# aosprey/mckpp-f90

Measured on AMD Instinct MI355X. Metric: column-steps/s at 1e5 cols x 60 levels, 1/2/4/8 GPU; % HBM roofline, higher is better.
Workload: dtype f64

## Files before the change

### mckpp_f90_amd/api.py

```python
import ctypes as C

import numpy as np

NI, NJ = 890, 48

F_PROFILES, F_SAVED, F_SCALARS, F_DIAG = 1, 2, 4, 8
F_RESTART = F_PROFILES | F_SAVED | F_SCALARS
F_ALL = 0xF

ST_ZERO_PIVOT, ST_LONG_ITER, ST_RETRIED, ST_FAILED, ST_DODGY = 1, 2, 4, 8, 16

_dp = C.POINTER(C.c_double)
_ip = C.POINTER(C.c_int32)

_SWITCHES = [
    "LKPP", "LRI", "LDD", "L_SSref", "L_RELAX_SST", "L_RELAX_CALCONLY", "L_FCORR", "L_FCORR_WITHZ",
    "L_SFCORR", "L_SFCORR_WITHZ", "L_RELAX_SAL", "L_RELAX_OCNT", "L_NO_FREEZE", "L_NO_ISOTHERM",
    "L_DAMP_CURR", "clim_present",
]


class _ConstC(C.Structure):
    _fields_ = (
        [(n, C.c_int32) for n in ("nz", "nztmax", "nsflxs", "njdt", "itermax")]
# ... 212 lines not shown
    "mckpp_hip_status": _sig(_H, _ip, _i64p, _ip, twin=True),
    "mckpp_hip_ncolumns": _sig(_H, res=_i64, twin=True),
    "mckpp_hip_last_kernel_ms": _sig(_H, _dp, _ip),
    "mckpp_hip_last_launch_count": _sig(_H, res=_i32),
    "mckpp_hip_kernel_name": _sig(_H, res=C.c_char_p),
    "mckpp_hip_kernel_residency": _sig(_H, _ip, _ip, _ip, _i64p),
    "mckpp_hip_eos_batch": _sig(_H, _i64, *[_dp] * 7),
    "mckpp_hip_exp_batch": _sig(_H, _i64, _dp, _dp),
    "mckpp_hip_div_batch": _sig(_H, _i64, _dp, _dp, _dp),
    "mckpp_hip_multi_ndev": _sig(_H, res=_i32),
    "mckpp_hip_multi_ctx": _sig(_H, _i32, res=_H),
    "mckpp_hip_multi_gather": _sig(_H, _i32, _i32, _dp),
}


def _signatures():
    out = {}
    for name, (res, argtypes, twin) in _SIGNATURES.items():
        out[name] = (res, argtypes)
        if twin:
            out["mckpp_hip_multi_" + name[len("mckpp_hip_"):]] = (res, argtypes)
    return out


def _bind(lib):
    if getattr(lib, "_mckpp_bound", False):
        return lib
    for name, (res, argtypes) in _signatures().items():
        fn = getattr(lib, name, None)
        if fn is not None:
            fn.restype, fn.argtypes = res, argtypes
    lib._mckpp_bound = True
    return lib


def _lib():
    from . import load_library

    return _bind(load_library())


def build_compiler():
    return _lib().mckpp_hip_build_compiler().decode()
# ... 406 lines not shown
        f = np.ascontiguousarray(fields, dtype=np.int32)
        self._call("window_select", f.ctypes.data_as(_ip), len(f))

    def window_fetch(self, field, op, out):
        assert out.flags["F_CONTIGUOUS"] and out.dtype == np.float64
        self._hold(out)
        self._call("window_fetch", int(field), int(op), out.ctypes.data_as(_dp))
        return out

    def set_diagnostics(self, on):
        self._call("set_diagnostics", int(on))

    def set_solver_mode(self, mode):
        self._call("set_solver_mode", int(mode))

    def init_ocean(self, ntime=0):
        self._call("init_ocean", int(ntime))

    def step(self, ntime, nsteps=1):
        self._call("step", int(ntime), int(nsteps))

    def synchronize(self):
        self._call("synchronize")

    def status(self):
        st = np.zeros(self._npts, dtype=np.int32)
        npass = np.zeros(self._npts, dtype=np.int32)
        nf = C.c_int64(0)
        self._call("status", st.ctypes.data_as(_ip), C.byref(nf), npass.ctypes.data_as(_ip))
        return st, int(nf.value), npass
# ... 66 lines not shown
        self._open(kpp_const_fields, len(dev), dev.ctypes.data_as(_ip))

    def gather(self, field, root, out):
        assert out.flags["F_CONTIGUOUS"] and out.dtype == np.float64
        self._hold(out)
        self._call("gather", int(field), int(root), out.ctypes.data_as(_dp))


def host_shard_mask(run_physics, ndev, dev):
    rp = np.ascontiguousarray(run_physics, dtype=np.int32)
    out = np.zeros(len(rp), dtype=np.int32)
    n = _lib().mckpp_host_shard_mask(len(rp), rp.ctypes.data_as(_ip), int(ndev), int(dev), out.ctypes.data_as(_ip))
    if n < 0:
        raise MckppHipError("mckpp_host_shard_mask: bad arguments")
    return out, int(n)


def _ctx(kpp_3d_fields, kpp_const_fields, device=0):
    ctx = getattr(kpp_const_fields, "_hip_ctx", None)
    if ctx is None:
        ctx = MckppHip(kpp_const_fields, device)
        kpp_const_fields._hip_ctx = ctx
        ctx._resident = None
    if ctx._resident is not kpp_3d_fields:
        ctx.upload(kpp_3d_fields)
        ctx._resident = kpp_3d_fields
    return ctx


def mckpp_initialize_ocean_model(kpp_3d_fields, kpp_const_fields, ntime=0, device=0, download=True):
# ... 18 lines not shown
```

### mckpp_f90_amd/csrc/mckpp_device.h

```cpp
#pragma once
#include <hip/hip_runtime.h>
#include <stdint.h>

#define MCKPP_CS 24
#define MCKPP_CI 8
#define MCKPP_XS 8
enum { XS_RELAX_SST = 0, XS_SST0, XS_FCORR_TWOD, XS_RELAX_SAL, XS_RELAX_OCNT };

enum {
  CS_F = 0, CS_SSURF, CS_SREF, CS_SSREF, CS_OCDEPTH,
  CS_SFLUX1, CS_SFLUX2, CS_SFLUX3, CS_SFLUX4, CS_SFLUX5, CS_SFLUX6,
  CS_HMIXD0, CS_HMIXD1, CS_HMIX, CS_KMIX, CS_UREF, CS_VREF, CS_TREF,
  CS_RESET, CS_DAMPU, CS_DAMPV, CS_FREEZE, CS_FCORR, CS_SPARE1
};
enum { CI_OLD = 0, CI_NEW, CI_JERLOV, CI_INITFLAG, CI_STATUS, CI_NPASS, CI_LOCEAN, CI_IPT };

enum { MCKPP_MODE_STEP = 0, MCKPP_MODE_INIT = 1, MCKPP_MODE_PASS = 2, MCKPP_MODE_VMIX = 3 };

template <class T> using mckpp_ptr_plain = T *;
template <class T> using mckpp_ptr_global = __attribute__((address_space(1))) T *;

#define MCKPP_WIN_ENTRIES 64
template <template <class> class P>
struct mckpp_win_t {
  P<const double> src;
  P<double> acc;
  long long plane;
  int ld, off, nlev, add_sref, ld_out;
  int ops, nops;
  int origin, period, nrec;
};

#define MCKPP_ANC_KINDS 7
enum { ANC_SST0 = 0, ANC_FCORR_TWOD, ANC_FCORR_WITHZ, ANC_SFCORR_WITHZ, ANC_OCNT_CLIM, ANC_SAL_CLIM, ANC_BOTTOM_TEMP };
struct mckpp_anc_sel { long long off_prev, off_next; double w_prev, w_next; };

typedef int mckpp_log_rec __attribute__((ext_vector_type(4)));

template <template <class> class P>
struct mckpp_kparams_t {
  int nz, nzp1, ncol, ld;
  int ntime, itermax, mode, diag;
  int L_SSref, LDD, clim_present;
  int l2pre;
  double hmixtolfrac, dto, grav, vonk, sice;
  double Vtc;
  double cg;
  double dm_nz;
  P<const double> zm, hm, tri0, tri1;
  P<const double> swfrac_tab;
  P<const double> swdk_tab;
  int ldc;
  int LRI;
  int solver_mode;
  int l3cap;
  int first_margin;
  int scan_rule;
  P<const double> wtab;
  P<double> U, V, T, S;
  P<double> Us[2], Vs[2], Ts[2], Ss[2];
  P<const double> U_init, V_init;
  P<double> cs;
  P<int> ci;
  P<int> qhead;
  int nsteps_launch;
  int nqueues;
  int xcc_queue[16];
  P<const double> series;
  int series_rec0, ndtocn, l_rest;
  int series_nring;
  double flsn, el;
  P<int> qowner;
  P<int> done;
  P<unsigned long long> dbg;
  int ext, L_RELAX_SST, L_RELAX_CALCONLY, L_FCORR, L_FCORR_WITHZ, L_SFCORR, L_SFCORR_WITHZ;
  int L_RELAX_SAL, L_RELAX_OCNT, L_NO_FREEZE, L_NO_ISOTHERM, L_DAMP_CURR, iso_bot, dt_uvdamp, maxmodeadv;
  double iso_thresh;
  P<const double> dm;
  P<const double> hsum;
  P<const double> xs;
  P<const double> fcorr_withz, sfcorr_withz, ocnT_clim, sal_clim;
// ... 22 lines not shown
  P<const double> anc_rec[MCKPP_ANC_KINDS];
  int anc_mask, anc_nt0;
  int diag_every;
};
#define MCKPP_SNAP_ROWS 14
using mckpp_kparams = mckpp_kparams_t<mckpp_ptr_plain>;
using mckpp_kparams_dev = mckpp_kparams_t<mckpp_ptr_global>;
using mckpp_win = mckpp_win_t<mckpp_ptr_plain>;
static_assert(sizeof(mckpp_kparams) == sizeof(mckpp_kparams_dev), "same layout");
static_assert(sizeof(mckpp_win) == sizeof(mckpp_win_t<mckpp_ptr_global>), "same layout");

struct mckpp_launch_info { int nblocks, threads, max_blocks_per_cu; size_t lds_bytes; };

hipError_t mckpp_launch_column_kernel_ps(const mckpp_kparams &p, const mckpp_kparams *dp, int num_cu,
                                         hipStream_t stream, mckpp_launch_info *info);
size_t mckpp_ps_scratch_doubles(int nzp1, int variant, int num_cu);
hipError_t mckpp_launch_xcc_probe(unsigned *mask, hipStream_t stream);
hipError_t mckpp_launch_eos_batch(int64_t n, const double *s, const double *t, const double *p,
                                  double *alpha, double *beta, double *sig0, double *cp,
                                  hipStream_t stream);
hipError_t mckpp_launch_div_batch(int64_t n, const double *num, const double *den, double *q, hipStream_t stream);
hipError_t mckpp_launch_exp_batch(int64_t n, const double *x, double *y, hipStream_t stream);
hipError_t mckpp_launch_bottomtemp(const mckpp_kparams &p, const double *bt, hipStream_t stream);
hipError_t mckpp_launch_fluxes(const mckpp_kparams &p, int ntime, const double *f8, int l_rest, double flsn,
                               double el, hipStream_t stream);
struct mckpp_pack_list { int nd, ni; int dslot[MCKPP_CS]; int islot[MCKPP_CI]; };
hipError_t mckpp_launch_unpack_sflux(const double *slabs, const int *ipt, double *cs, int64_t ncol, int64_t npts, hipStream_t stream);
hipError_t mckpp_launch_pack_records(const double *cs, const int *ci, const int *ipt, int64_t ncol, int64_t npts,
                                     const mckpp_pack_list &l, double *dout, int *iout, hipStream_t stream);
hipError_t mckpp_launch_out_sample(const double *src, int src_ld, int src_off, const double *cs, int add_sref,
// ... 18 lines not shown
```

### mckpp_f90_amd/csrc/mckpp_kernels_ps.hip

```cpp
#include "mckpp_colmath.h"

#include <cstdio>
#include <cstdlib>
#include <type_traits>

namespace {

using namespace mckpp_dev;

enum { PS_EMPTY = 0, PS_ACTIVE = 1, PS_DONE = 2, PS_WAIT = 3  };
enum { F_NONE = 0, F_TRAP = 1, F_FINAL = 2 };

enum {
  C_B0 = 0, C_B0SOL, C_USTAR, C_UFRAC, C_UCUBE, C_HEK, C_WU01, C_WU02, C_WX01, C_WX02, C_WXNT0, C_UREFNZ, C_VREFNZ,
  C_RHO0CP0, C_RRC, X_T1 , X_S1, X_RHOH2O, X_RHOB,
  C_F, C_HMIXE, C_HMIXN, C_HBL, C_RHBL, C_STABLE, C_BFSFC, C_CASEA,
  C_GAT1, C_DAT1 = C_GAT1 + 3, C_DKM1 = C_DAT1 + 3,
  C_SREF = C_DKM1 + 3, C_SSURF, C_OCDEPTH, C_SFLUX1, C_SFLUX2, C_SFLUX3, C_SFLUX4, C_SFLUX5, C_SFLUX6,
  C_T1X ,
  C_JRFAC = C_T1X + 2, C_JA1, C_JA2, C_JRA1, C_JRA2 ,
  C_COUNT_USED,
  C_COUNT = C_COUNT_USED | 1
};
enum {
  I_STATE = 0, I_ACT, I_COL, I_OLD, I_NEW, I_JER, I_INITFLAG, I_STATUS, I_NPASS, I_NPASS_TRY, I_ICONV, I_COMP, I_KMIXN,
// ... 859 lines not shown
  __device__ __forceinline__ double &operator[](int i) const { return b[i * KS]; }
};

template <int XV, int SM, int LF = 0>
#ifndef MCKPP_PS_MINW
#define MCKPP_PS_MINW 4
#endif
__global__ __launch_bounds__(1024, MCKPP_PS_MINW) void k_column_ps(const mckpp_kparams *__restrict__ pp, const int ntime, const int L_arg,
                                                     const int W0, const unsigned Lmagic_arg, const int SS )
{
  const int L = LF > 0 ? LF : L_arg;
  const unsigned Lmagic = LF > 0 ? (unsigned)(0x100000000ull / (unsigned long long)(LF > 0 ? LF : 1)) + 1u : Lmagic_arg;
  const mckpp_kparams_dev &p = *reinterpret_cast<const mckpp_kparams_dev *>(pp);
  extern __shared__ double lds[];
  constexpr bool EXT = XV != 0, DD = XV == 2;
  constexpr int ROWS = XV == 2 ? (int)Q_COUNT_EXT_DD : XV == 1 ? (int)Q_COUNT_EXT : (int)Q_COUNT;
  const int NL = ps_nl(L);
  const int tid = threadIdx.x, lane = tid & 63, lane_k = lane;
  const int wv = __builtin_amdgcn_readfirstlane(tid >> 6);
  const int nz = LF > 0 ? LF - 3 : p.nz, nzp1 = LF > 0 ? LF - 2 : p.nzp1;
  double *cst = lds;
  const strided<K_STRIDE> c_zm{cst + K_ZM}, c_hm{cst + K_HM}, c_t0{cst + K_T0}, c_t1{cst + K_T1}, c_rdz{cst + K_RDZ},
      c_dtohk{cst + K_DTOHK};
  double *c_misc = lds + K_STRIDE * NL;
  double *const slots0 = c_misc + 2;
  double *const screc0 = slots0 + W0 * SS;
  int *const sirec0 = reinterpret_cast<int *>(screc0 + W0 * C_COUNT);
  enum { S_KVIEW = 8, S_DRAIN = 9, S_GOVIEW = 10, S_MAP = 16, S_MAPMAX = 16 };
  int *s_flags = sirec0 + W0 * I_COUNT;
  const int W = W0;
// ... 108 lines not shown
    auto row = [&](int a) -> strided<ROWS> { return strided<ROWS>{my + a}; };             \
    (void)sc; (void)actz; (void)is1; (void)isnz; (void)row;

#ifdef MCKPP_PS_STAMPS
  int stamp_new = 0;
  unsigned long long gacc[6] = {0, 0, 0, 0, 0, 0};
#endif
  auto M0 = [&]() {
    int lane = lane_k; asm volatile("" : "+v"(lane));
    bool a = false, wt = false, sticky = false;
    const bool multi = p.nsteps_launch > 1;
    int *msi = sirec + (lane < W ? lane : 0) * I_COUNT;
    double *msc = screc + (lane < W ? lane : 0) * C_COUNT;
    int st = PS_DONE, c = 0, step = 0, kfirst = 0;
    bool want = false, ready = false, idle = false, dropped = false;
    bool cont = false;
    if (multi) {
      const bool pub = lane < W && msi[I_STATE] == PS_ACTIVE && msi[I_FIN] == F_FINAL;
      if (pub) {
        const int fc = msi[I_COL], fs = msi[I_STEP];
        int was = __hip_atomic_exchange(p.done + fc, fs + 1, __ATOMIC_RELAXED, __HIP_MEMORY_SCOPE_AGENT);
        asm volatile("s_waitcnt vmcnt(0)" : "+v"(was) : : "memory");
        if (fs + 1 < p.nsteps_launch) {
          const int q = fc % p.nqueues, nloc = (p.ncol - q + p.nqueues - 1) / p.nqueues;
          const int tnext = (fs + 1) * nloc + fc / p.nqueues;
          if (__hip_atomic_load((int *)p.qhead + q, __ATOMIC_RELAXED, __HIP_MEMORY_SCOPE_AGENT) > tnext)
            cont = atomicCAS((int *)p.done + p.ncol + fc, fs + 1, fs + 2) == fs + 1;
          if (cont) { c = fc; step = fs + 1; want = true; }
        }
      }
    }
    const bool any_cont = __ballot(cont) != 0ull;
    const int kv = solo_perm ? 0 : s_flags[S_KVIEW];
    const bool solo_on = kv > 0 && (any_cont || __ballot(lane < W && sirec[lane * I_COUNT + I_STATE] == PS_ACTIVE && sirec[lane * I_COUNT + I_FIN] != F_FINAL) != 0ull);
    if (lane < W) {
      st = msi[I_STATE];
      if (st == PS_ACTIVE && msi[I_FIN] == F_FINAL) st = PS_EMPTY;
      if (st == PS_WAIT && !solo_on) { c = msi[I_COL]; step = msi[I_STEP]; want = true; }
    }
    const int n_empty = __popcll(__ballot(lane < W && st == PS_EMPTY && !cont));
    const int n_busy = __popcll(__ballot(lane < W && st == PS_ACTIVE && sirec[lane * I_COUNT + I_NPASS_TRY] <= 12));
    bool refill = 2 * n_empty >= n_empty + n_busy;
    bool drain = false;
    if (p.solo_limit > 0 && p.mode == MCKPP_MODE_STEP) {
      const int after = p.solo_after;
      const bool was = lane < W && msi[I_STRAG] != 0;
      const bool gone = was && st != PS_ACTIVE;
      const bool is = lane < W && st == PS_ACTIVE && (was || msi[I_NPASS_TRY] > after);
      if (is && !was) msi[I_STRAG] = 1;
      if (gone) msi[I_STRAG] = 0;
      const int delta = __popcll(__ballot(is && !was)) - __popcll(__ballot(gone));
      int glob = 0;
      if (__ballot(is) != 0ull || delta != 0 || any_cont) {
        if (lane == 0) glob = delta != 0 ? atomicAdd((int *)p.sync, delta) + delta
                                         : __hip_atomic_load((int *)p.sync, __ATOMIC_RELAXED, __HIP_MEMORY_SCOPE_AGENT);
        glob = __shfl(glob, 0);
      }
      drain = (__ballot(is) != 0ull || any_cont) && glob <= p.solo_limit;
      if (solo_on) drain = true;
      else if (kv > 0 && lane == 0) s_flags[S_KVIEW] = 0;
      if (drain) refill = false;
    }
    if (lane < W) {
      if (st == PS_EMPTY) { msi[I_FIN] = F_NONE; msi[I_ACT] = 0; }
      if (st == PS_EMPTY && refill && !cont) {
        if (!multi) {
          const int t = atomicAdd((int *)p.qhead, 1);
          if (t >= p.ncol) { st = PS_DONE; msi[I_ACT] = 0; }
          else { c = t; want = true; }
        } else {
          msi[I_ACT] = 0;
          const int q = s_flags[7];
          const int nloc = q < 0 ? 0 : (p.ncol - q + p.nqueues - 1) / p.nqueues;
          for (;;) {
            const int t = nloc > 0 ? atomicAdd((int *)p.qhead + q, 1) : 0;
            if (nloc <= 0 || t >= nloc * p.nsteps_launch) { idle = true; break; }
            step = t / nloc;
            c = q + p.nqueues * (t - step * nloc);
            int *const started = (int *)p.done + p.ncol + c;
            if (__hip_atomic_load(started, __ATOMIC_RELAXED, __HIP_MEMORY_SCOPE_AGENT) > step) continue;
            if (step > 0 && __hip_atomic_load(p.done + c, __ATOMIC_RELAXED, __HIP_MEMORY_SCOPE_AGENT) < step) continue;
            if (atomicCAS(started, step, step + 1) != step) continue;
            want = true; ready = true;
            break;
          }
        }
      }
      if (cont || ready) ready = true;
      else if (want && multi) {
        int *const started = (int *)p.done + p.ncol + c;
        bool mine = false;
        if (__hip_atomic_load(started, __ATOMIC_RELAXED, __HIP_MEMORY_SCOPE_AGENT) <= step) {
          ready = step == 0 || __hip_atomic_load(p.done + c, __ATOMIC_RELAXED, __HIP_MEMORY_SCOPE_AGENT) >= step;
          mine = !ready || atomicCAS(started, step, step + 1) == step;
        }
        if (!mine) { want = false; ready = false; dropped = true; st = PS_EMPTY; msi[I_ACT] = 0; }
      } else if (want) ready = true;
    }
    if (multi && __ballot(want && ready && step > 0) != 0ull)
      __builtin_amdgcn_fence(__ATOMIC_ACQUIRE, "agent");
    bool more = false;
    if (multi && __ballot(idle) != 0ull) {
      int newq = -1;
      if (lane == 0) {
        for (int qq = 0; qq < p.nqueues && newq < 0; ++qq) {
          const int nl = (p.ncol - qq + p.nqueues - 1) / p.nqueues;
          if (nl <= 0 || __hip_atomic_load((int *)p.qhead + qq, __ATOMIC_RELAXED, __HIP_MEMORY_SCOPE_AGENT) >= nl * p.nsteps_launch) continue;
          const int prev = atomicCAS((int *)p.qowner + qq, 0, my_xcc + 1);
          if (prev == 0 || prev == my_xcc + 1) newq = qq;
        }
        s_flags[7] = newq;
      }
      more = __shfl(newq, 0) >= 0;
      if (idle && !more) st = PS_DONE;
    }
    if (lane < W) {
      if (want && !ready) {
        st = PS_WAIT;
        msi[I_ACT] = 0; msi[I_COL] = c; msi[I_STEP] = step;
      } else if (want) {
        {
          st = PS_ACTIVE;
// ... 242 lines not shown
        msi[I_FIN] = fin;
        msi[I_L1A] = (l1_ahead && fin == F_NONE) ? 1 : 0;
        f_any = fin != F_NONE;
      }
    }
    const unsigned long long m = __ballot(f_any);
    if (lane == 0) s_flags[1] = m != 0ull ? 1 : 0;
#ifdef MCKPP_PS_STAMPS
    {
      const bool sg = lane < W && sirec[lane * I_COUNT + I_STATE] == PS_ACTIVE && sirec[lane * I_COUNT + I_ACT] && sirec[lane * I_COUNT + I_STRAG];
      const int n = __popcll(__ballot(sg));
      const int nact = __popcll(__ballot(lane < W && sirec[lane * I_COUNT + I_STATE] == PS_ACTIVE && sirec[lane * I_COUNT + I_ACT]));
      if (lane == 0 && n > 0) { atomicAdd((int *)p.sync + (sparse ? 1 : 2), n); atomicAdd((int *)p.sync + (sparse ? 3 : 4), 1); atomicAdd((int *)p.sync + (sparse ? 5 : 6), nact); }
    }
#endif
    if (solo_dyn && !sparse) {
      const int f_kv = s_flags[S_KVIEW], f_drain = s_flags[S_DRAIN];
      if (f_kv == 0 && f_drain) {
        const int *msi = sirec + (lane < W ? lane : 0) * I_COUNT;
        const bool on = lane < W && msi[I_STATE] == PS_ACTIVE && msi[I_ACT];
        const bool ok = on && msi[I_FIN] == F_NONE && (msi[I_STRAG] || msi[I_NPASS_TRY] > p.solo_after);
        const unsigned long long m_on = __ballot(on), m_ok = __ballot(ok);
        const int kn = __popcll(m_on);
        if (kn >= 1 && kn <= kmax_view && m_ok == m_on) {
          if (on) s_flags[S_MAP + __popcll(m_on & ((1ull << lane) - 1ull))] = lane;
          if (lane == 0) s_flags[S_GOVIEW] = kn;
        }
      }
    }
  };
  auto G_late = [&]() {
    int lane = lane_k; asm volatile("" : "+v"(lane));
    if (lane < W) {
      int *msi = sirec + lane * I_COUNT;
      if (msi[I_ACT]) {
        if (p.mode != MCKPP_MODE_INIT && msi[I_BAD]) msi[I_STATUS] = msi[I_STATUS] | 1;
        msi[I_BAD] = 0;
        msi[I_TINY] = 0;
        msi[I_MAYBE] = msi[I_MAYBE_NEXT];
// ... 1175 lines not shown
      if (max_slots_per_cu && b * w > *max_slots_per_cu) *max_slots_per_cu = b * w;
    }
  }
  return g;
}

}

size_t mckpp_ps_scratch_doubles(int nzp1, int xv, int num_cu)
{
  int most = 1;
  (void)ps_geometry(nzp1 + 2, xv, 1 << 20, &most);
  return (size_t)num_cu * most * 4 * ps_scratch_ld(nzp1);
}

hipError_t mckpp_launch_column_kernel_ps(const mckpp_kparams &p, const mckpp_kparams *dp, int num_cu, hipStream_t stream,
                                         mckpp_launch_info *info)
{
  if (p.ncol <= 0) return hipSuccess;
  const int L = p.nzp1 + 2;
  if (L > 1024) return hipErrorInvalidValue;
  const int xv = p.ext ? (p.LDD ? 2 : 1) : 0;
  const ps_geom g = ps_geometry(L, xv, (p.ncol + num_cu - 1) / num_cu, nullptr);
  if (!p.scratch || p.scratch_doubles < (size_t)num_cu * g.per_cu * g.w * 4 * ps_scratch_ld(p.nzp1)) return hipErrorInvalidValue;
  const size_t lds = ps_lds_bytes(L, g.w, xv);
  if (lds > (size_t)160 * 1024) return hipErrorInvalidValue;
  using kern_t = void (*)(const mckpp_kparams *, int, int, int, unsigned, int);
  static const kern_t kerns_63[2] = {k_column_ps<0, 0, 63>, k_column_ps<0, 1, 63>}, kerns_72[2] = {k_column_ps<0, 0, 72>, k_column_ps<0, 1, 72>},
                      kerns_103[2] = {k_column_ps<0, 0, 103>, k_column_ps<0, 1, 103>};
  static const kern_t kernx_63[2] = {k_column_ps<1, 0, 63>, k_column_ps<1, 1, 63>}, kernx_72[2] = {k_column_ps<1, 0, 72>, k_column_ps<1, 1, 72>},
                      kernx_103[2] = {k_column_ps<1, 0, 103>, k_column_ps<1, 1, 103>};
  static const kern_t kerns[2][3] = {{k_column_ps<0, 0>, k_column_ps<1, 0>, k_column_ps<2, 0>},
                                     {k_column_ps<0, 1>, k_column_ps<1, 1>, k_column_ps<2, 1>}};
  if (p.solver_mode < 0 || p.solver_mode > 1) return hipErrorInvalidValue;
  const bool fixed_l = !(getenv("MCKPP_PS_FIXED_L") && atoi(getenv("MCKPP_PS_FIXED_L")) == 0);
  const kern_t kern = (fixed_l && xv == 0 && L == 63) ? kerns_63[p.solver_mode] : (fixed_l && xv == 0 && L == 72) ? kerns_72[p.solver_mode]
                    : (fixed_l && xv == 0 && L == 103) ? kerns_103[p.solver_mode]
                    : (fixed_l && xv == 1 && L == 63) ? kernx_63[p.solver_mode] : (fixed_l && xv == 1 && L == 72) ? kernx_72[p.solver_mode]
                    : (fixed_l && xv == 1 && L == 103) ? kernx_103[p.solver_mode] : kerns[p.solver_mode][xv];
  const void *fn = reinterpret_cast<const void *>(kern);
  hipError_t e = hipFuncSetAttribute(fn, hipFuncAttributeMaxDynamicSharedMemorySize, (int)lds);
  if (e != hipSuccess) return e;
  int nblocks = num_cu * g.per_cu;
  const int groups = (p.ncol + g.w - 1) / g.w;
  if (nblocks > groups) nblocks = groups;
  if (nblocks < 1) nblocks = 1;
  if (info) {
    int nb = 0;
    if (hipOccupancyMaxActiveBlocksPerMultiprocessor(&nb, fn, 64 * g.nw, lds) != hipSuccess) nb = 0;
    *info = {nblocks, 64 * g.nw, nb, lds};
// ... 16 lines not shown
```

### mckpp_f90_amd/csrc/mckpp_runtime.cpp

```cpp
#include "../../include/mckpp_hip.h"
#include "mckpp_device.h"
#include "mckpp_math.h"
#include "mckpp_own.h"

#include <algorithm>
#include <cmath>
#include <cstdarg>
#include <cstdio>
#include <cstdlib>
#include <cstring>
#include <exception>
#include <functional>
#include <string>
#include <thread>
#include <vector>

namespace {

thread_local std::string g_err;

int fail(const char *fmt, ...)
{
  char buf[512];
  va_list ap;
// ... 31 lines not shown
}

enum { P_U = 0, P_V, P_T, P_S, P_US0, P_US1, P_VS0, P_VS1, P_TS0, P_TS1, P_SS0, P_SS1, P_UINIT, P_VINIT, P_COUNT };
enum { E_FCORR_WITHZ = 0, E_SFCORR_WITHZ, E_OCNT_CLIM, E_SAL_CLIM, E_COUNT };
enum { O_TINC = 0, O_SINC, O_OCNTCORR, O_SCORR, O_COUNT };
enum { D_RHO = 0, D_CP, D_BUOY, D_TALPHA, D_SBETA, D_DIFM, D_DIFS, D_DIFT, D_GHAT, D_WU1, D_WU2,
       D_WX1, D_WX2, D_WX3, D_WXNT1, D_RIG, D_DBLOC, D_SHSQ, D_COUNT };

const double jer_rfac[6] = {0, 0.58, 0.62, 0.67, 0.77, 0.78};
const double jer_a1[6] = {0, 0.35, 0.6, 1.0, 1.5, 1.4};
const double jer_a2[6] = {0, 23.0, 20.0, 17.0, 14.0, 7.9};

}

enum { QBLOCK_INTS = 64 };
enum { FIRST_MARGIN_DEFAULT = 12, GUESS_MARGIN_DEFAULT = 0 };

struct mckpp_ctx_streams {
  hip_stream stream;
  hip_stream copy_stream;
  hip_stream snap_stream;
  hip_stream flux_stream;
};

struct mckpp_ctx_resident {
  int64_t npts = 0, ncol = 0;
  dev_buf<int> d_ipt;
  dev_buf<double> d_prof[P_COUNT];
  dev_buf<double> d_diag[D_COUNT];
  dev_buf<double> d_ext_in[E_COUNT];
// ... 79 lines not shown
  dev_buf<double2> d_wtab;
  std::vector<int> ipt;
  bool ext = false;
  bool ext_kernel = false;
  std::vector<int> wsel{0, 1, 2, 3, 4};
  dev_buf<mckpp_win> d_win;
  dev_buf<mckpp_anc_sel> d_anc_sel;
  pinned_turns<mckpp_anc_sel> h_anc_sel;
  int anc_mask = 0, anc_nt0 = 0;
  pinned_buf<char> h_snap[2];
  hip_event ev_snap[2];
  dev_buf<int> d_qhead;
  int view_kmax = 0;
  int solo_after = 12, solo_limit = 8;
  bool multistep = true;
  int nqueues = 0;
  int xcc_queue[16];
  int l3cap = 0;
  int first_guess = 1, first_margin = FIRST_MARGIN_DEFAULT, guess_margin = GUESS_MARGIN_DEFAULT;
  int solver_mode = 0;
  dev_buf<unsigned long long> d_dbg;
  dev_buf<mckpp_kparams> d_params;
  pinned_turns<mckpp_kparams> h_params;
  dev_buf<double> d_scratch;
  size_t scratch_doubles = 0;
  int num_cu = 256;
  int l2pre = 0;
  mckpp_launch_info last_launch{};
  hip_event ev_lay[2], ev_copy[2];
  unsigned xfer_seq = 0;
// ... 43 lines not shown
      if (zehat >= 0.) {
        wm = vonk * usta / (1. + c1 * zeta);
        ws = wm;
      } else {
        wm = (zeta > zetam) ? vonk * usta * std::pow(1. - c2 * zeta, 1. / 4.)
                            : vonk * std::pow(am * u3 - cm * zehat, 1. / 3.);
        ws = (zeta > zetas) ? vonk * usta * std::sqrt(1. - c3 * zeta)
                            : vonk * std::pow(as * u3 - cs * zehat, 1. / 3.);
      }
      wmt[(size_t)j * n1 + i] = wm;
      wst[(size_t)j * n1 + i] = ws;
    }
  }
}

void mckpp_host_tri(int32_t nz, int32_t nztmax, double dto, const double *zm, const double *hm, double *tri)
{
  const int n1 = nztmax + 1;
  auto Z = [&](int k) { return zm[k - 1]; };
  auto H = [&](int k) { return hm[k - 1]; };
  double *t0 = tri, *t1 = tri + n1;
  for (int k = 0; k < n1; ++k) { t0[k] = 0.0; t1[k] = 0.0; }
  t1[0] = dto / H(1);
  t1[1] = dto / H(1) / (Z(1) - Z(2));
  for (int k = 2; k <= nz; ++k) {
    t1[k] = dto / H(k) / (Z(k) - Z(k + 1));
    t0[k] = dto / H(k) / (Z(k - 1) - Z(k));
  }
}

// ... 36 lines not shown
  h->ldc = 64 * lpl + 8;
  h->num_cu = prop.multiProcessorCount;
  h->ext = c->LDD || c->L_RELAX_SST || c->L_FCORR || c->L_FCORR_WITHZ || c->L_SFCORR || c->L_SFCORR_WITHZ ||
           c->L_RELAX_SAL || c->L_RELAX_OCNT || c->L_NO_FREEZE || c->L_NO_ISOTHERM || c->L_DAMP_CURR ||
           c->clim_present || c->L_ADVECT;
  h->ext_kernel = c->LDD || c->L_RELAX_SST || c->L_FCORR || c->L_FCORR_WITHZ || c->L_SFCORR || c->L_SFCORR_WITHZ ||
                  c->L_RELAX_SAL || c->L_RELAX_OCNT || c->L_NO_FREEZE || c->L_NO_ISOTHERM || c->L_DAMP_CURR || c->L_ADVECT;
  HIPCHK(h->stream.create());
  HIPCHK(h->d_qhead.alloc(QBLOCK_INTS));
  h->solo_after = 12;
  h->solo_limit = std::max(2, h->num_cu / 32);
  if (const char *e = getenv("MCKPP_SOLO")) { if (atoi(e) == 0) h->solo_limit = 0; }
  if (const char *e = getenv("MCKPP_SOLO_LIMIT")) h->solo_limit = std::max(0, atoi(e));
  if (const char *e = getenv("MCKPP_SOLO_AFTER")) h->solo_after = std::max(0, atoi(e));
  if (const char *e = getenv("MCKPP_VIEW_KMAX")) h->view_kmax = std::max(0, atoi(e));
  {
    HIPCHK(hipMemsetAsync(h->d_qhead, 0, sizeof(int), h->stream));
    HIPCHK(mckpp_launch_xcc_probe(reinterpret_cast<unsigned *>(h->d_qhead.get()), h->stream));
    unsigned mask = 0;
    HIPCHK(hipMemcpyAsync(&mask, h->d_qhead, sizeof mask, hipMemcpyDeviceToHost, h->stream));
    HIPCHK(hipStreamSynchronize(h->stream));
    h->nqueues = 0;
    for (int i = 0; i < 16; ++i) h->xcc_queue[i] = (mask >> i & 1u) ? h->nqueues++ : -1;
    if (h->nqueues == 0) h->multistep = false;
    if (const char *e = getenv("MCKPP_XCC_DROP")) {
      const unsigned drop = (unsigned)strtoul(e, nullptr, 0);
      for (int i = 0; i < 16; ++i) if (drop >> i & 1u) h->xcc_queue[i] = -1;
    }
    if (getenv("MCKPP_PS_VERBOSE"))
      fprintf(stderr, "[mckpp] XCC ids seen by the probe: mask 0x%x, %d queues\n", mask, h->nqueues);
// ... 680 lines not shown
  if (!h) return fail("null handle");
  h->diag = on ? 1 : 0;
  return 0;
}

int mckpp_hip_set_solver_mode(mckpp_hip_handle h, int mode)
{
  if (!h) return fail("null handle");
  if (mode < 0 || mode > 1) return fail("mckpp_hip_set_solver_mode: unknown solver mode (0: the reference's order, 1: two-ended)");
  h->solver_mode = mode;
  return 0;
}

int mckpp_hip_get_solver_mode(mckpp_hip_handle h) { return h ? h->solver_mode : fail("null handle"); }

static bool win_is_diag(int f) { return f >= MCKPP_OUT_B && f <= MCKPP_OUT_SINC_FCORR; }

static void fill_params(mckpp_hip_ctx *h, mckpp_kparams &p, int ntime, int mode)
{
  memset(&p, 0, sizeof p);
  p.nz = h->nz; p.nzp1 = h->nzp1; p.ncol = (int)h->ncol; p.ld = h->ld;
  p.ntime = ntime; p.itermax = h->c.itermax; p.mode = mode; p.diag = h->diag;
  p.L_SSref = h->c.L_SSref; p.LDD = h->c.LDD; p.clim_present = h->c.clim_present;
  p.l2pre = h->l2pre; p.LRI = h->c.LRI ? 1 : 0; p.l3cap = h->l3cap;
  p.first_margin = h->first_guess ? h->first_margin : -1; p.scan_rule = h->guess_margin | (h->first_guess ? 1 << 16 : 0);
  p.solver_mode = h->solver_mode;
  p.hmixtolfrac = h->c.hmixtolfrac; p.dto = h->c.dto; p.grav = h->c.grav; p.vonk = h->c.vonk; p.sice = h->c.sice;
  p.Vtc = h->Vtc; p.cg = h->cg; p.dm_nz = h->dm_nz;
  p.zm = h->d_zm; p.hm = h->d_hm; p.tri0 = h->d_tri0; p.tri1 = h->d_tri1;
  p.swfrac_tab = h->d_swfrac_tab; p.swdk_tab = h->d_swdk_tab; p.ldc = h->ldc; p.wtab = reinterpret_cast<const double *>(h->d_wtab.get());
  p.U = h->d_prof[P_U]; p.V = h->d_prof[P_V]; p.T = h->d_prof[P_T]; p.S = h->d_prof[P_S];
  p.Us[0] = h->d_prof[P_US0]; p.Us[1] = h->d_prof[P_US1]; p.Vs[0] = h->d_prof[P_VS0]; p.Vs[1] = h->d_prof[P_VS1];
  p.Ts[0] = h->d_prof[P_TS0]; p.Ts[1] = h->d_prof[P_TS1]; p.Ss[0] = h->d_prof[P_SS0]; p.Ss[1] = h->d_prof[P_SS1];
  p.U_init = h->d_prof[P_UINIT]; p.V_init = h->d_prof[P_VINIT];
  p.cs = h->d_cs; p.ci = h->d_ci; p.qhead = h->d_qhead; p.dbg = h->d_dbg;
  p.nsteps_launch = 1; p.done = h->d_done; p.nqueues = h->nqueues; p.qowner = h->d_qhead + 16;
  p.sync = h->d_qhead + 32; p.solo_after = h->solo_after; p.solo_limit = h->solo_limit; p.view_kmax = h->view_kmax;
  for (int i = 0; i < 16; ++i) p.xcc_queue[i] = h->xcc_queue[i];
  p.ext = h->ext_kernel ? 1 : 0;
  p.L_RELAX_SST = h->c.L_RELAX_SST; p.L_RELAX_CALCONLY = h->c.L_RELAX_CALCONLY; p.L_FCORR = h->c.L_FCORR;
  p.L_FCORR_WITHZ = h->c.L_FCORR_WITHZ; p.L_SFCORR = h->c.L_SFCORR; p.L_SFCORR_WITHZ = h->c.L_SFCORR_WITHZ;
  p.L_RELAX_SAL = h->c.L_RELAX_SAL; p.L_RELAX_OCNT = h->c.L_RELAX_OCNT; p.L_NO_FREEZE = h->c.L_NO_FREEZE;
  p.L_NO_ISOTHERM = h->c.L_NO_ISOTHERM; p.L_DAMP_CURR = h->c.L_DAMP_CURR; p.iso_bot = h->c.iso_bot;
  p.dt_uvdamp = h->c.dt_uvdamp; p.maxmodeadv = h->c.maxmodeadv; p.iso_thresh = h->c.iso_thresh;
  p.dm = h->d_dm; p.hsum = h->d_hsum; p.xs = h->d_xs; p.adv_i = h->d_adv_i; p.adv_d = h->d_adv_d;
  p.fcorr_withz = h->d_ext_in[E_FCORR_WITHZ]; p.sfcorr_withz = h->d_ext_in[E_SFCORR_WITHZ];
  p.ocnT_clim = h->d_ext_in[E_OCNT_CLIM]; p.sal_clim = h->d_ext_in[E_SAL_CLIM];
  p.tinc_fcorr = h->d_ext_out[O_TINC]; p.sinc_fcorr = h->d_ext_out[O_SINC];
  p.ocnTcorr = h->d_ext_out[O_OCNTCORR]; p.scorr = h->d_ext_out[O_SCORR];
  p.rho = h->d_diag[D_RHO]; p.cp = h->d_diag[D_CP]; p.buoy = h->d_diag[D_BUOY];
  p.talpha = h->d_diag[D_TALPHA]; p.sbeta = h->d_diag[D_SBETA];
// ... 69 lines not shown
    fill_params(h, *q, ntime, mode);
    HIPCHK(hipMemcpyAsync(h->d_params, q, sizeof(mckpp_kparams), hipMemcpyHostToDevice, h->stream));
    HIPCHK(h->h_params.queued(h->stream));
  }
  HIPCHK(hipEventRecord(h->ev0, h->stream));
  if (mode == MCKPP_MODE_STEP && nsteps > 1 && ntime >= 1 && h->multistep) {
    if (!h->d_done) HIPCHK(h->d_done.alloc(2 * (size_t)h->ncol));
    const int per_launch = (int)std::max<int64_t>(1, ((int64_t)1 << 30) / h->ncol);
    for (int i = 0; i < nsteps; i += per_launch) {
      const int n = nsteps - i < per_launch ? nsteps - i : per_launch;
      mckpp_kparams *qp = nullptr;
      HIPCHK(h->h_params.take(1, &qp));
      mckpp_kparams &q = *qp;
      fill_params(h, q, ntime + i, mode);
      q.nsteps_launch = n;
      if (forced) {
        q.series = forced->series; q.series_rec0 = forced->rec0; q.series_nring = forced->nring;
        q.ndtocn = forced->ndtocn; q.l_rest = forced->l_rest;
        q.flsn = forced->flsn; q.el = forced->el;
      }
      HIPCHK(hipMemcpyAsync(h->d_params, qp, sizeof(mckpp_kparams), hipMemcpyHostToDevice, h->stream));
      HIPCHK(h->h_params.queued(h->stream));
      HIPCHK(hipMemsetAsync(h->d_qhead, 0, QBLOCK_INTS * sizeof(int), h->stream));
      HIPCHK(hipMemsetAsync(h->d_done, 0, 2 * (size_t)h->ncol * sizeof(int), h->stream));
      HIPCHK(mckpp_launch_column_kernel_ps(q, h->d_params, h->num_cu, h->stream, &h->last_launch));
    }
    HIPCHK(hipEventRecord(h->ev1, h->stream));
    h->nlaunch = nsteps;
    h->nkernels = (nsteps + per_launch - 1) / per_launch;
    h->timed = true;
// ... 1601 lines not shown
  }
  m->gipt_valid = false;
  return 0;
}

#define MULTI_EACH(call)                                           \
  do {                                                             \
    if (!m) return fail("null multi handle");                      \
    for (auto *x : m->ctx) { if ((call) != 0) return -1; }         \
    return 0;                                                      \
  } while (0)

int mckpp_hip_multi_set_forcing(mckpp_hip_multi_handle m, const double *sflux) { MULTI_EACH(mckpp_hip_set_forcing(x, sflux)); }
int mckpp_hip_multi_set_diagnostics(mckpp_hip_multi_handle m, int on) { MULTI_EACH(mckpp_hip_set_diagnostics(x, on)); }
int mckpp_hip_multi_set_solver_mode(mckpp_hip_multi_handle m, int mode) { MULTI_EACH(mckpp_hip_set_solver_mode(x, mode)); }
int mckpp_hip_multi_init_ocean(mckpp_hip_multi_handle m, int ntime) { MULTI_EACH(mckpp_hip_init_ocean(x, ntime)); }
int mckpp_hip_multi_step(mckpp_hip_multi_handle m, int ntime, int nsteps) { MULTI_EACH(mckpp_hip_step(x, ntime, nsteps)); }
int mckpp_hip_multi_synchronize(mckpp_hip_multi_handle m) { MULTI_EACH(mckpp_hip_synchronize(x)); }
int mckpp_hip_multi_update_ancillaries(mckpp_hip_multi_handle m, const mckpp_state_ptrs_c *s) { MULTI_EACH(mckpp_hip_update_ancillaries(x, s)); }
int mckpp_hip_multi_bottomtemp(mckpp_hip_multi_handle m, const double *bottom_temp) { MULTI_EACH(mckpp_hip_bottomtemp(x, bottom_temp)); }
int mckpp_hip_multi_set_bottomtemp(mckpp_hip_multi_handle m, const double *bottom_temp) { MULTI_EACH(mckpp_hip_set_bottomtemp(x, bottom_temp)); }
int mckpp_hip_multi_set_ancillary_series(mckpp_hip_multi_handle m, int kind, int rec0, int nrec, const double *records)
{
  MULTI_EACH(mckpp_hip_set_ancillary_series(x, kind, rec0, nrec, records));
}
int mckpp_hip_multi_ancillary_schedule(mckpp_hip_multi_handle m, int kind, int nt_origin, int cadence, int epoch0, int nepochs,
                                       const mckpp_anc_epoch_c *epochs)
{
  MULTI_EACH(mckpp_hip_ancillary_schedule(x, kind, nt_origin, cadence, epoch0, nepochs, epochs));
}
// ... 538 lines not shown
```

Before: 36.97 million.

## Hand out multi-step tickets in step chunks so columns continue across steps

```diff
diff --git a/include/mckpp_hip_sched.h b/include/mckpp_hip_sched.h
--- /dev/null
+++ b/include/mckpp_hip_sched.h
@@ -0,0 +1,18 @@
+#ifndef MCKPP_HIP_SCHED_H
+#define MCKPP_HIP_SCHED_H
+#include "mckpp_hip.h"
+
+#ifdef __cplusplus
+extern "C" {
+#endif
+
+int mckpp_hip_set_step_chunk(mckpp_hip_handle h, int chunk);
+int mckpp_hip_multi_set_step_chunk(mckpp_hip_multi_handle m, int chunk);
+
+int mckpp_host_tickets(int32_t ncol, int32_t nqueues, int32_t nsteps, int32_t chunk, int32_t q, int32_t *out);
+int mckpp_host_ticket_at(int32_t ncol, int32_t nqueues, int32_t nsteps, int32_t chunk, int32_t col, int32_t step);
+
+#ifdef __cplusplus
+}
+#endif
+#endif
diff --git a/mckpp_f90_amd/api.py b/mckpp_f90_amd/api.py
--- a/mckpp_f90_amd/api.py
+++ b/mckpp_f90_amd/api.py
@@ -250,19 +250,30 @@
 }
 
 
-def _signatures():
+_SCHED_SIGNATURES = {
+    "mckpp_hip_set_step_chunk": _sig(_H, _i, twin=True),
+    "mckpp_host_tickets": _sig(_i32, _i32, _i32, _i32, _i32, _ip),
+    "mckpp_host_ticket_at": _sig(_i32, _i32, _i32, _i32, _i32, _i32),
+}
+
+
+def _spell_out(table):
     out = {}
-    for name, (res, argtypes, twin) in _SIGNATURES.items():
+    for name, (res, argtypes, twin) in table.items():
         out[name] = (res, argtypes)
         if twin:
             out["mckpp_hip_multi_" + name[len("mckpp_hip_"):]] = (res, argtypes)
     return out
 
 
+def _signatures():
+    return _spell_out(_SIGNATURES)
+
+
 def _bind(lib):
     if getattr(lib, "_mckpp_bound", False):
         return lib
-    for name, (res, argtypes) in _signatures().items():
+    for name, (res, argtypes) in {**_signatures(), **_spell_out(_SCHED_SIGNATURES)}.items():
         fn = getattr(lib, name, None)
         if fn is not None:
             fn.restype, fn.argtypes = res, argtypes
@@ -699,6 +710,9 @@
     def set_solver_mode(self, mode):
         self._call("set_solver_mode", int(mode))
 
+    def set_step_chunk(self, chunk):
+        self._call("set_step_chunk", int(chunk))
+
     def init_ocean(self, ntime=0):
         self._call("init_ocean", int(ntime))
 
@@ -795,6 +809,23 @@
     if n < 0:
         raise MckppHipError("mckpp_host_shard_mask: bad arguments")
     return out, int(n)
+
+
+def host_tickets(ncol, nqueues, nsteps, chunk, q):
+    lib = _lib()
+    n = lib.mckpp_host_tickets(int(ncol), int(nqueues), int(nsteps), int(chunk), int(q), None)
+    _chk(0 if n >= 0 else n)
+    out = np.zeros((n, 3), dtype=np.int32)
+    if n:
+        lib.mckpp_host_tickets(int(ncol), int(nqueues), int(nsteps), int(chunk), int(q), out.ctypes.data_as(_ip))
+    return out
+
+
+def host_ticket_at(ncol, nqueues, nsteps, chunk, col, step):
+    t = _lib().mckpp_host_ticket_at(int(ncol), int(nqueues), int(nsteps), int(chunk), int(col), int(step))
+    if t < -1:
+        raise MckppHipError("mckpp_host_ticket_at: bad arguments")
+    return int(t)
 
 
 def _ctx(kpp_3d_fields, kpp_const_fields, device=0):
diff --git a/mckpp_f90_amd/csrc/mckpp_device.h b/mckpp_f90_amd/csrc/mckpp_device.h
--- a/mckpp_f90_amd/csrc/mckpp_device.h
+++ b/mckpp_f90_amd/csrc/mckpp_device.h
@@ -37,6 +37,21 @@
 
 typedef int mckpp_log_rec __attribute__((ext_vector_type(4)));
 
+struct mckpp_ticket { int j, step, len; };
+__host__ __device__ inline int mckpp_queue_columns(int ncol, int nqueues, int q) { return (ncol - q + nqueues - 1) / nqueues; }
+__host__ __device__ inline int mckpp_ticket_count(int nloc, int nsteps, int chunk) { return nloc * (1 + (nsteps - 1 + chunk - 1) / chunk); }
+__host__ __device__ inline mckpp_ticket mckpp_ticket_of(int t, int nloc, int nsteps, int chunk)
+{
+  const int k = t / nloc, s = k == 0 ? 0 : 1 + (k - 1) * chunk;
+  return {t - k * nloc, s, k == 0 ? 1 : (nsteps - s < chunk ? nsteps - s : chunk)};
+}
+__host__ __device__ inline int mckpp_ticket_at(int j, int step, int nloc, int chunk)
+{
+  if (step == 0) return j;
+  const int k = (step - 1) / chunk;
+  return step - 1 == k * chunk ? (1 + k) * nloc + j : -1;
+}
+
 template <template <class> class P>
 struct mckpp_kparams_t {
   int nz, nzp1, ncol, ld;
@@ -65,6 +80,7 @@
   P<int> qhead;
   int nsteps_launch;
   int nqueues;
+  int step_chunk;
   int xcc_queue[16];
   P<const double> series;
   int series_rec0, ndtocn, l_rest;
@@ -117,6 +133,7 @@
 
 hipError_t mckpp_launch_column_kernel_ps(const mckpp_kparams &p, const mckpp_kparams *dp, int num_cu,
                                          hipStream_t stream, mckpp_launch_info *info);
+int mckpp_ps_slots(int nzp1, int variant, int num_cu, int ncol);
 size_t mckpp_ps_scratch_doubles(int nzp1, int variant, int num_cu);
 hipError_t mckpp_launch_xcc_probe(unsigned *mask, hipStream_t stream);
 hipError_t mckpp_launch_eos_batch(int64_t n, const double *s, const double *t, const double *p,
diff --git a/mckpp_f90_amd/csrc/mckpp_kernels_ps.hip b/mckpp_f90_amd/csrc/mckpp_kernels_ps.hip
--- a/mckpp_f90_amd/csrc/mckpp_kernels_ps.hip
+++ b/mckpp_f90_amd/csrc/mckpp_kernels_ps.hip
@@ -8,7 +8,8 @@
 
 using namespace mckpp_dev;
 
-enum { PS_EMPTY = 0, PS_ACTIVE = 1, PS_DONE = 2, PS_WAIT = 3  };
+enum { PS_EMPTY = 0, PS_ACTIVE = 1, PS_DONE = 2, PS_WAIT = 3 ,
+       PS_HOLD = 4  };
 enum { F_NONE = 0, F_TRAP = 1, F_FINAL = 2 };
 
 enum {
@@ -898,6 +899,7 @@
   const mckpp_kparams_dev &p = *reinterpret_cast<const mckpp_kparams_dev *>(pp);
   extern __shared__ double lds[];
   constexpr bool EXT = XV != 0, DD = XV == 2;
+  constexpr bool CH = LF != 103;
   constexpr int ROWS = XV == 2 ? (int)Q_COUNT_EXT_DD : XV == 1 ? (int)Q_COUNT_EXT : (int)Q_COUNT;
   const int NL = ps_nl(L);
   const int tid = threadIdx.x, lane = tid & 63, lane_k = lane;
@@ -1036,19 +1038,26 @@
     double *msc = screc + (lane < W ? lane : 0) * C_COUNT;
     int st = PS_DONE, c = 0, step = 0, kfirst = 0;
     bool want = false, ready = false, idle = false, dropped = false;
-    bool cont = false;
+    bool cont = false, hold = false;
     if (multi) {
       const bool pub = lane < W && msi[I_STATE] == PS_ACTIVE && msi[I_FIN] == F_FINAL;
       if (pub) {
         const int fc = msi[I_COL], fs = msi[I_STEP];
         int was = __hip_atomic_exchange(p.done + fc, fs + 1, __ATOMIC_RELAXED, __HIP_MEMORY_SCOPE_AGENT);
-        asm volatile("s_waitcnt vmcnt(0)" : "+v"(was) : : "memory");
+        if constexpr (!CH) asm volatile("s_waitcnt vmcnt(0)" : "+v"(was) : : "memory");
         if (fs + 1 < p.nsteps_launch) {
-          const int q = fc % p.nqueues, nloc = (p.ncol - q + p.nqueues - 1) / p.nqueues;
-          const int tnext = (fs + 1) * nloc + fc / p.nqueues;
-          if (__hip_atomic_load((int *)p.qhead + q, __ATOMIC_RELAXED, __HIP_MEMORY_SCOPE_AGENT) > tnext)
-            cont = atomicCAS((int *)p.done + p.ncol + fc, fs + 1, fs + 2) == fs + 1;
-          if (cont) { c = fc; step = fs + 1; want = true; }
+          const int q = fc % p.nqueues, nloc = mckpp_queue_columns(p.ncol, p.nqueues, q);
+          int tnext;
+          if constexpr (CH) tnext = mckpp_ticket_at(fc / p.nqueues, fs + 1, nloc, p.step_chunk);
+          else tnext = (fs + 1) * nloc + fc / p.nqueues;
+          if (CH && tnext < 0) {
+            hold = true; c = fc; step = fs + 1;
+          } else {
+            if constexpr (CH) asm volatile("s_waitcnt vmcnt(0)" : "+v"(was) : : "memory");
+            if (__hip_atomic_load((int *)p.qhead + q, __ATOMIC_RELAXED, __HIP_MEMORY_SCOPE_AGENT) > tnext)
+              cont = atomicCAS((int *)p.done + p.ncol + fc, fs + 1, fs + 2) == fs + 1;
+            if (cont) { c = fc; step = fs + 1; want = true; }
+          }
         }
       }
     }
@@ -1059,10 +1068,12 @@
       st = msi[I_STATE];
       if (st == PS_ACTIVE && msi[I_FIN] == F_FINAL) st = PS_EMPTY;
       if (st == PS_WAIT && !solo_on) { c = msi[I_COL]; step = msi[I_STEP]; want = true; }
+      if (CH && st == PS_HOLD) { hold = true; c = msi[I_COL]; step = msi[I_STEP]; st = PS_EMPTY; }
     }
     const int n_empty = __popcll(__ballot(lane < W && st == PS_EMPTY && !cont));
     const int n_busy = __popcll(__ballot(lane < W && st == PS_ACTIVE && sirec[lane * I_COUNT + I_NPASS_TRY] <= 12));
     bool refill = 2 * n_empty >= n_empty + n_busy;
+    const bool round = refill;
     bool drain = false;
     if (p.solo_limit > 0 && p.mode == MCKPP_MODE_STEP) {
       const int after = p.solo_after;
@@ -1085,7 +1096,14 @@
     }
     if (lane < W) {
       if (st == PS_EMPTY) { msi[I_FIN] = F_NONE; msi[I_ACT] = 0; }
-      if (st == PS_EMPTY && refill && !cont) {
+      if (CH && hold) {
+        if (round) {
+          __hip_atomic_store((int *)p.done + p.ncol + c, step + 1, __ATOMIC_RELAXED, __HIP_MEMORY_SCOPE_AGENT);
+          want = true; ready = true;
+        } else {
+          st = PS_HOLD; msi[I_COL] = c; msi[I_STEP] = step;
+        }
+      } else if (st == PS_EMPTY && refill && !cont) {
         if (!multi) {
           const int t = atomicAdd((int *)p.qhead, 1);
           if (t >= p.ncol) { st = PS_DONE; msi[I_ACT] = 0; }
@@ -1093,12 +1111,19 @@
         } else {
           msi[I_ACT] = 0;
           const int q = s_flags[7];
-          const int nloc = q < 0 ? 0 : (p.ncol - q + p.nqueues - 1) / p.nqueues;
+          const int nloc = q < 0 ? 0 : mckpp_queue_columns(p.ncol, p.nqueues, q);
+          const int ntickets = CH ? mckpp_ticket_count(nloc, p.nsteps_launch, p.step_chunk) : nloc * p.nsteps_launch;
           for (;;) {
             const int t = nloc > 0 ? atomicAdd((int *)p.qhead + q, 1) : 0;
-            if (nloc <= 0 || t >= nloc * p.nsteps_launch) { idle = true; break; }
-            step = t / nloc;
-            c = q + p.nqueues * (t - step * nloc);
+            if (nloc <= 0 || t >= ntickets) { idle = true; break; }
+            if constexpr (CH) {
+              const mckpp_ticket tk = mckpp_ticket_of(t, nloc, p.nsteps_launch, p.step_chunk);
+              step = tk.step;
+              c = q + p.nqueues * tk.j;
+            } else {
+              step = t / nloc;
+              c = q + p.nqueues * (t - step * nloc);
+            }
             int *const started = (int *)p.done + p.ncol + c;
             if (__hip_atomic_load(started, __ATOMIC_RELAXED, __HIP_MEMORY_SCOPE_AGENT) > step) continue;
             if (step > 0 && __hip_atomic_load(p.done + c, __ATOMIC_RELAXED, __HIP_MEMORY_SCOPE_AGENT) < step) continue;
@@ -1126,8 +1151,8 @@
       int newq = -1;
       if (lane == 0) {
         for (int qq = 0; qq < p.nqueues && newq < 0; ++qq) {
-          const int nl = (p.ncol - qq + p.nqueues - 1) / p.nqueues;
-          if (nl <= 0 || __hip_atomic_load((int *)p.qhead + qq, __ATOMIC_RELAXED, __HIP_MEMORY_SCOPE_AGENT) >= nl * p.nsteps_launch) continue;
+          const int nl = mckpp_queue_columns(p.ncol, p.nqueues, qq);
+          if (nl <= 0 || __hip_atomic_load((int *)p.qhead + qq, __ATOMIC_RELAXED, __HIP_MEMORY_SCOPE_AGENT) >= (CH ? mckpp_ticket_count(nl, p.nsteps_launch, p.step_chunk) : nl * p.nsteps_launch)) continue;
           const int prev = atomicCAS((int *)p.qowner + qq, 0, my_xcc + 1);
           if (prev == 0 || prev == my_xcc + 1) newq = qq;
         }
@@ -1400,6 +1425,14 @@
       if (lane == 0 && n > 0) { atomicAdd((int *)p.sync + (sparse ? 1 : 2), n); atomicAdd((int *)p.sync + (sparse ? 3 : 4), 1); atomicAdd((int *)p.sync + (sparse ? 5 : 6), nact); }
     }
 #endif
+    if constexpr (CH) {
+      if (p.nsteps_launch > 1 && !sparse) {
+        const int *hsi = sirec + (lane < W ? lane : 0) * I_COUNT;
+        const bool held = lane < W && hsi[I_STATE] == PS_HOLD;
+        const bool busy = lane < W && hsi[I_STATE] == PS_ACTIVE && hsi[I_NPASS_TRY] <= 12;
+        if (__ballot(held) != 0ull && __ballot(busy) == 0ull && lane == 0) s_flags[6] = 1;
+      }
+    }
     if (solo_dyn && !sparse) {
       const int f_kv = s_flags[S_KVIEW], f_drain = s_flags[S_DRAIN];
       if (f_kv == 0 && f_drain) {
@@ -1408,7 +1441,8 @@
         const bool ok = on && msi[I_FIN] == F_NONE && (msi[I_STRAG] || msi[I_NPASS_TRY] > p.solo_after);
         const unsigned long long m_on = __ballot(on), m_ok = __ballot(ok);
         const int kn = __popcll(m_on);
-        if (kn >= 1 && kn <= kmax_view && m_ok == m_on) {
+        const bool held = CH && __ballot(lane < W && msi[I_STATE] == PS_HOLD) != 0ull;
+        if (kn >= 1 && kn <= kmax_view && m_ok == m_on && !held) {
           if (on) s_flags[S_MAP + __popcll(m_on & ((1ull << lane) - 1ull))] = lane;
           if (lane == 0) s_flags[S_GOVIEW] = kn;
         }
@@ -2614,6 +2648,14 @@
   return (size_t)num_cu * most * 4 * ps_scratch_ld(nzp1);
 }
 
+int mckpp_ps_slots(int nzp1, int xv, int num_cu, int ncol)
+{
+  if (ncol <= 0) return 0;
+  const ps_geom g = ps_geometry(nzp1 + 2, xv, (ncol + num_cu - 1) / num_cu, nullptr);
+  const int groups = (ncol + g.w - 1) / g.w;
+  return std::max(1, std::min(num_cu * g.per_cu, groups)) * g.w;
+}
+
 hipError_t mckpp_launch_column_kernel_ps(const mckpp_kparams &p, const mckpp_kparams *dp, int num_cu, hipStream_t stream,
                                          mckpp_launch_info *info)
 {
@@ -2633,7 +2675,8 @@
   static const kern_t kerns[2][3] = {{k_column_ps<0, 0>, k_column_ps<1, 0>, k_column_ps<2, 0>},
                                      {k_column_ps<0, 1>, k_column_ps<1, 1>, k_column_ps<2, 1>}};
   if (p.solver_mode < 0 || p.solver_mode > 1) return hipErrorInvalidValue;
-  const bool fixed_l = !(getenv("MCKPP_PS_FIXED_L") && atoi(getenv("MCKPP_PS_FIXED_L")) == 0);
+  bool fixed_l = !(getenv("MCKPP_PS_FIXED_L") && atoi(getenv("MCKPP_PS_FIXED_L")) == 0);
+  if (L == 103 && p.nsteps_launch > 1 && p.step_chunk > 1) fixed_l = false;
   const kern_t kern = (fixed_l && xv == 0 && L == 63) ? kerns_63[p.solver_mode] : (fixed_l && xv == 0 && L == 72) ? kerns_72[p.solver_mode]
                     : (fixed_l && xv == 0 && L == 103) ? kerns_103[p.solver_mode]
                     : (fixed_l && xv == 1 && L == 63) ? kernx_63[p.solver_mode] : (fixed_l && xv == 1 && L == 72) ? kernx_72[p.solver_mode]
diff --git a/mckpp_f90_amd/csrc/mckpp_runtime.cpp b/mckpp_f90_amd/csrc/mckpp_runtime.cpp
--- a/mckpp_f90_amd/csrc/mckpp_runtime.cpp
+++ b/mckpp_f90_amd/csrc/mckpp_runtime.cpp
@@ -1,4 +1,5 @@
 #include "../../include/mckpp_hip.h"
+#include "../../include/mckpp_hip_sched.h"
 #include "mckpp_device.h"
 #include "mckpp_math.h"
 #include "mckpp_own.h"
@@ -69,6 +70,11 @@
 }
 
 enum { QBLOCK_INTS = 64 };
+static int step_chunk_default(int nzp1, int variant, int num_cu, int64_t ncol)
+{
+  if ((nzp1 + 2 != 63 && nzp1 + 2 != 72) || variant == 2) return 1;
+  return ncol >= 12 * (int64_t)mckpp_ps_slots(nzp1, variant, num_cu, ncol > INT32_MAX ? INT32_MAX : (int)ncol) ? 4 : 1;
+}
 enum { FIRST_MARGIN_DEFAULT = 12, GUESS_MARGIN_DEFAULT = 0 };
 
 struct mckpp_ctx_streams {
@@ -178,6 +184,7 @@
   int view_kmax = 0;
   int solo_after = 12, solo_limit = 8;
   bool multistep = true;
+  int step_chunk = 0, step_chunk_env = 0;
   int nqueues = 0;
   int xcc_queue[16];
   int l3cap = 0;
@@ -251,6 +258,23 @@
   }
 }
 
+int mckpp_host_tickets(int32_t ncol, int32_t nqueues, int32_t nsteps, int32_t chunk, int32_t q, int32_t *out)
+{
+  if (ncol < 1 || nqueues < 1 || nsteps < 1 || chunk < 1 || q < 0 || q >= nqueues) return fail("mckpp_host_tickets: bad argument");
+  const int nloc = mckpp_queue_columns(ncol, nqueues, q), n = mckpp_ticket_count(nloc, nsteps, chunk);
+  for (int t = 0; out && t < n; ++t) {
+    const mckpp_ticket tk = mckpp_ticket_of(t, nloc, nsteps, chunk);
+    out[3 * t] = q + nqueues * tk.j; out[3 * t + 1] = tk.step; out[3 * t + 2] = tk.len;
+  }
+  return n;
+}
+
+int mckpp_host_ticket_at(int32_t ncol, int32_t nqueues, int32_t nsteps, int32_t chunk, int32_t col, int32_t step)
+{
+  if (ncol < 1 || nqueues < 1 || nsteps < 1 || chunk < 1 || col < 0 || col >= ncol || step < 0 || step >= nsteps) return -2;
+  return mckpp_ticket_at(col / nqueues, step, mckpp_queue_columns(ncol, nqueues, col % nqueues), chunk);
+}
+
 void mckpp_host_tri(int32_t nz, int32_t nztmax, double dto, const double *zm, const double *hm, double *tri)
 {
   const int n1 = nztmax + 1;
@@ -317,6 +341,10 @@
   if (const char *e = getenv("MCKPP_SOLO_LIMIT")) h->solo_limit = std::max(0, atoi(e));
   if (const char *e = getenv("MCKPP_SOLO_AFTER")) h->solo_after = std::max(0, atoi(e));
   if (const char *e = getenv("MCKPP_VIEW_KMAX")) h->view_kmax = std::max(0, atoi(e));
+  if (const char *e = getenv("MCKPP_STEP_CHUNK")) {
+    if (atoi(e) < 1) return fail("mckpp_hip_init: MCKPP_STEP_CHUNK=%s (steps per ticket of a multi-step launch: at least 1)", e);
+    h->step_chunk_env = atoi(e);
+  }
   {
     HIPCHK(hipMemsetAsync(h->d_qhead, 0, sizeof(int), h->stream));
     HIPCHK(mckpp_launch_xcc_probe(reinterpret_cast<unsigned *>(h->d_qhead.get()), h->stream));
@@ -1027,6 +1055,14 @@
 
 int mckpp_hip_get_solver_mode(mckpp_hip_handle h) { return h ? h->solver_mode : fail("null handle"); }
 
+int mckpp_hip_set_step_chunk(mckpp_hip_handle h, int chunk)
+{
+  if (!h) return fail("null handle");
+  if (chunk < 1) return fail("mckpp_hip_set_step_chunk: chunk=%d (steps per ticket of a multi-step launch: at least 1)", chunk);
+  h->step_chunk = chunk;
+  return 0;
+}
+
 static bool win_is_diag(int f) { return f >= MCKPP_OUT_B && f <= MCKPP_OUT_SINC_FCORR; }
 
 static void fill_params(mckpp_hip_ctx *h, mckpp_kparams &p, int ntime, int mode)
@@ -1047,7 +1083,7 @@
   p.Ts[0] = h->d_prof[P_TS0]; p.Ts[1] = h->d_prof[P_TS1]; p.Ss[0] = h->d_prof[P_SS0]; p.Ss[1] = h->d_prof[P_SS1];
   p.U_init = h->d_prof[P_UINIT]; p.V_init = h->d_prof[P_VINIT];
   p.cs = h->d_cs; p.ci = h->d_ci; p.qhead = h->d_qhead; p.dbg = h->d_dbg;
-  p.nsteps_launch = 1; p.done = h->d_done; p.nqueues = h->nqueues; p.qowner = h->d_qhead + 16;
+  p.nsteps_launch = 1; p.step_chunk = 1; p.done = h->d_done; p.nqueues = h->nqueues; p.qowner = h->d_qhead + 16;
   p.sync = h->d_qhead + 32; p.solo_after = h->solo_after; p.solo_limit = h->solo_limit; p.view_kmax = h->view_kmax;
   for (int i = 0; i < 16; ++i) p.xcc_queue[i] = h->xcc_queue[i];
   p.ext = h->ext_kernel ? 1 : 0;
@@ -1147,6 +1183,9 @@
       mckpp_kparams &q = *qp;
       fill_params(h, q, ntime + i, mode);
       q.nsteps_launch = n;
+      const int chunk = h->step_chunk_env > 0 ? h->step_chunk_env : h->step_chunk > 0 ? h->step_chunk
+                      : step_chunk_default(h->nzp1, h->ext_kernel ? (h->c.LDD ? 2 : 1) : 0, h->num_cu, h->ncol);
+      q.step_chunk = std::min(n, chunk);
       if (forced) {
         q.series = forced->series; q.series_rec0 = forced->rec0; q.series_nring = forced->nring;
         q.ndtocn = forced->ndtocn; q.l_rest = forced->l_rest;
@@ -2778,6 +2817,7 @@
 int mckpp_hip_multi_set_forcing(mckpp_hip_multi_handle m, const double *sflux) { MULTI_EACH(mckpp_hip_set_forcing(x, sflux)); }
 int mckpp_hip_multi_set_diagnostics(mckpp_hip_multi_handle m, int on) { MULTI_EACH(mckpp_hip_set_diagnostics(x, on)); }
 int mckpp_hip_multi_set_solver_mode(mckpp_hip_multi_handle m, int mode) { MULTI_EACH(mckpp_hip_set_solver_mode(x, mode)); }
+int mckpp_hip_multi_set_step_chunk(mckpp_hip_multi_handle m, int chunk) { MULTI_EACH(mckpp_hip_set_step_chunk(x, chunk)); }
 int mckpp_hip_multi_init_ocean(mckpp_hip_multi_handle m, int ntime) { MULTI_EACH(mckpp_hip_init_ocean(x, ntime)); }
 int mckpp_hip_multi_step(mckpp_hip_multi_handle m, int ntime, int nsteps) { MULTI_EACH(mckpp_hip_step(x, ntime, nsteps)); }
 int mckpp_hip_multi_synchronize(mckpp_hip_multi_handle m) { MULTI_EACH(mckpp_hip_synchronize(x)); }
```

Result: faster. 37.80 million, median of 6 (+2.3%).
